# Advanced-Vision-and-Learning-Lab/sparse-view-3dgs-pack

Hardware: AMD Instinct MI355X
Metric: train-step views/s (fwd+bwd) @1M Gaussians 1080p (higher is better)
Workload: dtype f32

## Files before the change

include/gsplat.h:

```cpp
#ifndef GSPLAT_H_INCLUDED
#define GSPLAT_H_INCLUDED

#include <stddef.h>
#include <stdint.h>

#ifdef __cplusplus
extern "C" {
#endif

#define GS_ABI_VERSION 7

#define GS_OK 0
#define GS_E_NULL (-1)
#define GS_E_SHAPE (-2)
#define GS_E_SCRATCH (-3)
#define GS_E_OVERFLOW (-4)
#define GS_E_UNSUPPORTED (-5)

#define GS_TILE_X 16
#define GS_TILE_Y 16
#define GS_NUM_CHANNELS 3

typedef struct GsView {
  int32_t image_height;
// ... 66 lines not shown
int gs_scratch_bytes(int32_t P, int32_t W, int32_t H, int64_t R_capacity, size_t out[3],
                     size_t* backward_workspace_bytes);

int gs_forward_geometry(const GsView* view, const GsGaussians* g, GsScratch* scratch,
                        int32_t* radii, int32_t* num_rendered_host, void* stream);

int gs_forward_render(const GsView* view, const GsGaussians* g, GsScratch* scratch,
                      float* out_color, float* out_invdepth, void* stream);

int gs_forward_bin(const GsView* view, const GsGaussians* g, GsScratch* scratch, uint32_t* status_host, void* stream);

int gs_forward_render_x(const GsView* view, const GsGaussians* g, GsScratch* scratch,
                        float* out_color, float* out_invdepth, float* out_extra, void* stream);

int gs_backward(const GsView* view, const GsGaussians* g, const int32_t* radii,
                const GsScratch* scratch, int64_t num_rendered, const float* dL_dcolor,
                const float* dL_dinvdepth, const GsGrads* grads, void* workspace,
                size_t workspace_bytes, void* stream);

int gs_backward_x(const GsView* view, const GsGaussians* g, const int32_t* radii,
                  const GsScratch* scratch, int64_t num_rendered, const float* dL_dcolor,
                  const float* dL_dinvdepth, const float* dL_dextra_img, const GsGrads* grads,
                  void* workspace, size_t workspace_bytes, void* stream);

int gs_forward_render_fsgs(const GsView* view, const GsGaussians* g, GsScratch* scratch,
                           float* out_color, float* out_depth, float* out_alpha, void* stream);
int gs_backward_fsgs(const GsView* view, const GsGaussians* g, const int32_t* radii,
                     const GsScratch* scratch, int64_t num_rendered, const float* dL_dcolor,
                     const float* dL_ddepth, const float* dL_dalpha, const GsGrads* grads,
                     void* workspace, size_t workspace_bytes, void* stream);

int gs_mark_visible(int32_t P, const float* means3D, const float* viewmatrix,
                    const float* projmatrix, uint8_t* present, void* stream);

int gs_export_geom(const GsScratch* scratch, int32_t P, float* depths, float* means2D ,
                   float* cov3D , float* conic_opacity , float* rgb ,
                   uint8_t* clamped , uint32_t* tiles_touched, uint32_t* point_offsets,
                   void* stream);
int gs_export_binning(const GsScratch* scratch, int64_t num_rendered, uint64_t* keys_sorted,
                      uint32_t* point_list, void* stream);
int gs_export_img(const GsScratch* scratch, int32_t W, int32_t H, float* final_T,
                  uint32_t* n_contrib, uint32_t* ranges , void* stream);

typedef struct GsStepState {
  float* xyz;
  float* features;
  float* opacity;
  float* scaling;
  float* rotation;
  float* m[5];
  float* v[5];
  float lr[6];
  int32_t step[5];
  float beta1, beta2, eps;
  float* max_radii2D;
  float* xyz_gradient_accum;
  float* denom;
  const float* coef_dev;
  const double* rows_override;
  float* grad_out[5];
  float* fail_flag;
  int32_t phase;
  int32_t rows_clean;
  void* phase1_done;
  float* extra;
  float* extra_m;
// ... 237 lines not shown
```

sparse-view-3dgs-pack_amd/csrc/gs_preprocess.hip:

```cpp
#include "gs_common.h"
#include "gs_tilecull.h"
#include "gs_math.h"

template <typename SH>
GS_DEV V3 color_from_sh(int deg, V3 pos, V3 campos, const SH& sh, uint32_t& clamped) {
  V3 dir = pos - campos;
  dir = dir / length3(dir);
  V3 result = SH_C0 * sh(0);
  if (deg > 0) {
    float x = dir.x, y = dir.y, z = dir.z;
    result = result - SH_C1 * y * sh(1) + SH_C1 * z * sh(2) - SH_C1 * x * sh(3);
    if (deg > 1) {
      float xx = x * x, yy = y * y, zz = z * z;
      float xy = x * y, yz = y * z, xz = x * z;
      result = result + SH_C2_0 * xy * sh(4) + SH_C2_1 * yz * sh(5) + SH_C2_2 * (2.0f * zz - xx - yy) * sh(6) +
               SH_C2_3 * xz * sh(7) + SH_C2_4 * (xx - yy) * sh(8);
      if (deg > 2) {
        result = result + SH_C3_0 * y * (3.0f * xx - yy) * sh(9) + SH_C3_1 * xy * z * sh(10) +
                 SH_C3_2 * y * (4.0f * zz - xx - yy) * sh(11) + SH_C3_3 * z * (2.0f * zz - 3.0f * xx - 3.0f * yy) * sh(12) +
                 SH_C3_4 * x * (4.0f * zz - xx - yy) * sh(13) + SH_C3_5 * z * (xx - yy) * sh(14) +
                 SH_C3_6 * x * (xx - 3.0f * yy) * sh(15);
      }
    }
  }
// ... 2 lines not shown
  result.z += 0.5f;
  clamped = (result.x < 0 ? 1u : 0u) | (result.y < 0 ? 2u : 0u) | (result.z < 0 ? 4u : 0u);
  return {fmaxf(result.x, 0.0f), fmaxf(result.y, 0.0f), fmaxf(result.z, 0.0f)};
}

struct ShRegs {
  float f[48];
  __device__ __forceinline__ V3 operator()(int k) const { return {f[3 * k], f[3 * k + 1], f[3 * k + 2]}; }
};
struct ShMem {
  const float* p;
  __device__ __forceinline__ V3 operator()(int k) const { return {p[3 * k], p[3 * k + 1], p[3 * k + 2]}; }
};
struct ShMemSplit {
  const float *dc, *rest;
  __device__ __forceinline__ V3 operator()(int k) const {
    const float* p = k == 0 ? dc : rest + 3 * (k - 1);
    return {p[0], p[1], p[2]};
  }
};

#ifndef GS_LIMIT_TILES_IN_LDS
#define GS_LIMIT_TILES_IN_LDS 0
#endif
#define GS_LIMIT_LDS_MAX_FLOATS (GS_LIMIT_TILES_IN_LDS ? 10240 : 4096)
extern __shared__ float s_limit[];
static inline size_t preprocess_limit_lds_floats(const PreprocessArgs& a) {
  if (!a.tile_depth_limit) return 0;
  const size_t T = (size_t)a.grid_x * a.grid_y, all = depth_limit_floats((uint32_t)a.grid_x, (uint32_t)a.grid_y);
  const size_t want = GS_LIMIT_TILES_IN_LDS ? all : all - T;
  return want <= GS_LIMIT_LDS_MAX_FLOATS ? want : 0;
}

__global__ void __launch_bounds__(GS_BLOCK) preprocess_fwd_kernel(PreprocessArgs a, GeomView g, int lds_floats) {
  const int idx = blockIdx.x * GS_BLOCK + threadIdx.x;
  uint32_t tiles = 0, entries = TB_ENTRIES_UNKNOWN;
  const int T = a.grid_x * a.grid_y;
  int p0 = 0, p1 = 0, p2 = 0, p3 = 0, n_pend = 0;
  uint32_t s0 = 0xFFFFFFFFu, s1 = 0xFFFFFFFFu, s2 = 0xFFFFFFFFu, s3 = 0xFFFFFFFFu, dbits = 0;
  auto bump = [&]() {
    if (n_pend > 0) s0 = atomicAdd(&a.region_count[(size_t)p0 * RG_COUNT_STRIDE], 1u);
    if (n_pend > 1) s1 = atomicAdd(&a.region_count[(size_t)p1 * RG_COUNT_STRIDE], 1u);
    if (n_pend > 2) s2 = atomicAdd(&a.region_count[(size_t)p2 * RG_COUNT_STRIDE], 1u);
    if (n_pend > 3) s3 = atomicAdd(&a.region_count[(size_t)p3 * RG_COUNT_STRIDE], 1u);
    n_pend = 0;
  };
  auto collect = [&]() {
    const uint2 entry = make_uint2(dbits, (uint32_t)idx);
    if (s0 < a.region_cap) a.region_bucket[(size_t)p0 * a.region_cap + s0] = entry;
    if (s1 < a.region_cap) a.region_bucket[(size_t)p1 * a.region_cap + s1] = entry;
    if (s2 < a.region_cap) a.region_bucket[(size_t)p2 * a.region_cap + s2] = entry;
    if (s3 < a.region_cap) a.region_bucket[(size_t)p3 * a.region_cap + s3] = entry;
    s0 = s1 = s2 = s3 = 0xFFFFFFFFu;
  };
  const int lidx = min(idx, a.P - 1);
  typedef const __attribute__((address_space(4))) float* GsConstFloatPtr;
  float vm[16], pm[16], cam[3];
  {
    const GsConstFloatPtr vmp = (GsConstFloatPtr)(uintptr_t)a.viewmatrix, pmp = (GsConstFloatPtr)(uintptr_t)a.projmatrix;
    const GsConstFloatPtr cp = (GsConstFloatPtr)(uintptr_t)a.campos;
#pragma unroll
    for (int k = 0; k < 16; k++) { vm[k] = vmp[k]; pm[k] = pmp[k]; }
    cam[0] = cp[0]; cam[1] = cp[1]; cam[2] = cp[2];
  }
  const bool own_cov = a.cov3D_precomp == nullptr;
  const float* sc_p = own_cov ? a.scales + 3 * (size_t)lidx : a.cov3D_precomp + 6 * (size_t)lidx;
  const float* rq_p = own_cov ? a.rotations + 4 * (size_t)lidx : a.cov3D_precomp + 6 * (size_t)lidx;
  float op_in = a.opacities[lidx];
  V3 p_orig = {a.means3D[3 * (size_t)lidx], a.means3D[3 * (size_t)lidx + 1], a.means3D[3 * (size_t)lidx + 2]};
  V3 sc_in = {sc_p[0], sc_p[1], sc_p[2]};
  V4 rq_in = {rq_p[0], rq_p[1], rq_p[2], rq_p[3]};
  if (lds_floats) {
    const float* src = a.tile_depth_limit + (GS_LIMIT_TILES_IN_LDS ? 0 : T);
    for (int i = threadIdx.x; i < lds_floats; i += GS_BLOCK) s_limit[i] = src[i];
    __syncthreads();
  }
  asm volatile("" : "+v"(op_in), "+v"(sc_in.x), "+v"(sc_in.y), "+v"(sc_in.z), "+v"(rq_in.x), "+v"(rq_in.y), "+v"(rq_in.z),
               "+v"(rq_in.w));
  const GsLdsFloatPtr lds_seg = (GsLdsFloatPtr)s_limit + (GS_LIMIT_TILES_IN_LDS ? T : 0);
  if (idx == 0) g.hdr->pad[HDR_LIMITED] = a.tile_depth_limit ? 1u : 0u;
  if (idx < a.P) {
    Splat sp;
    sp.x = sp.y = sp.depth = sp.invdepth = 0.f;
    sp.cxx = sp.cxy = sp.cyy = sp.opacity = 0.f;
    sp.r = sp.g = sp.b = 0.f;
    sp.extra = 0.f;
    int radius_out = 0;
    sp.rect_min = sp.rect_max = sp.tiles = sp.clamped = 0;
    float cov3D[6] = {0, 0, 0, 0, 0, 0};
    bool write_cov = false;
    do {
      V3 p_view = xform4x3(p_orig, vm);
      if (p_view.z <= 0.2f) break;
      V4 p_hom = xform4x4(p_orig, pm);
      float p_w = 1.0f / (p_hom.w + 0.0000001f);
      V3 p_proj = {p_hom.x * p_w, p_hom.y * p_w, p_hom.z * p_w};

      if (a.cov3D_precomp != nullptr) {
#pragma unroll
        for (int k = 0; k < 6; k++) cov3D[k] = a.cov3D_precomp[(size_t)idx * 6 + k];
      } else {
        const V3 sc = activate_scales(sc_in, a.raw_activations);
        const V4 rq = activate_rotation(rq_in, a.raw_activations);
        M3 S = mat3_cols(1, 0, 0, 0, 1, 0, 0, 0, 1);
        S.c[0][0] = a.scale_modifier * sc.x;
        S.c[1][1] = a.scale_modifier * sc.y;
        S.c[2][2] = a.scale_modifier * sc.z;
        M3 R = quat_to_R(rq);
        M3 Mm = mul3(S, R);
        M3 Sigma = mul3(transpose3(Mm), Mm);
        cov3D[0] = Sigma.c[0][0];
        cov3D[1] = Sigma.c[0][1];
        cov3D[2] = Sigma.c[0][2];
        cov3D[3] = Sigma.c[1][1];
        cov3D[4] = Sigma.c[1][2];
        cov3D[5] = Sigma.c[2][2];
        write_cov = true;
      }
      Cov2DInter ci;
      cov2d_common(p_orig, a.focal_x, a.focal_y, a.tan_fovx, a.tan_fovy, cov3D, vm, ci);
      M3 cv = mul3(mul3(transpose3(ci.T), transpose3(ci.Vrk)), ci.T);
      V3 cov = {cv.c[0][0], cv.c[0][1], cv.c[1][1]};

      const float h_var = 0.3f;
      const float det_cov = cov.x * cov.z - cov.y * cov.y;
      cov.x += h_var;
      cov.z += h_var;
      const float det_cov_plus_h_cov = cov.x * cov.z - cov.y * cov.y;
      float h_convolution_scaling = 1.0f;
      if (a.antialiasing) h_convolution_scaling = sqrtf(fmaxf(0.000025f, det_cov / det_cov_plus_h_cov));
      const float det = det_cov_plus_h_cov;
      if (det == 0.0f) break;
      float det_inv = 1.f / det;
      V3 conic = {cov.z * det_inv, -cov.y * det_inv, cov.x * det_inv};
      float mid = 0.5f * (cov.x + cov.z);
      float lambda1 = mid + sqrtf(fmaxf(0.1f, mid * mid - det));
      float lambda2 = mid - sqrtf(fmaxf(0.1f, mid * mid - det));
      float my_radius = ceilf(3.f * sqrtf(fmaxf(lambda1, lambda2)));
      float pix_x = ndc2pix(p_proj.x, a.W), pix_y = ndc2pix(p_proj.y, a.H);
      uint32_t minx, miny, maxx, maxy;
      const int radius_i = f2i_sat(my_radius);
      get_rect(pix_x, pix_y, radius_i, a.grid_x, a.grid_y, minx, miny, maxx, maxy);
      if ((maxx - minx) * (maxy - miny) == 0) break;

      sp.depth = p_view.z;
      sp.invdepth = 1 / p_view.z;
      radius_out = radius_i;
      sp.extra = a.extra_channel ? load_extra(a.extra_channel, a.extra_gain, idx, a.raw_activations) : 0.f;
      sp.x = pix_x;
      sp.y = pix_y;
      sp.cxx = conic.x; sp.cxy = conic.y; sp.cyy = conic.z;
      sp.opacity = activate_opacity(op_in, a.raw_activations) * h_convolution_scaling;
      sp.rect_min = minx | (miny << 16);
      sp.rect_max = maxx | (maxy << 16);
      if (a.tile_cull == 2) {
        const TileCull tc = tilecull_setup(1, sp.x, sp.y, sp.cxx, sp.cxy, sp.cyy, sp.opacity);
        if (tc.mode != 1) {
          int tx0 = (int)minx, tx1 = (int)maxx, ty0 = (int)miny, ty1 = (int)maxy;
          if (tc.mode == 2) {
            const float big = 1.0e6f;
            const float xl = fminf(fmaxf(sp.x - tc.ex - 1.0f, -big), big), xh = fminf(fmaxf(sp.x + tc.ex + 1.0f, -big), big);
            const float yl = fminf(fmaxf(sp.y - tc.ey - 1.0f, -big), big), yh = fminf(fmaxf(sp.y + tc.ey + 1.0f, -big), big);
            tx0 = max(tx0, (int)floorf(xl * 0.0625f));
            tx1 = min(tx1, (int)floorf(xh * 0.0625f) + 1);
            ty0 = max(ty0, (int)floorf(yl * 0.0625f));
            ty1 = min(ty1, (int)floorf(yh * 0.0625f) + 1);
          }
          if (tx1 > tx0 && ty1 > ty0) {
            const int segs_x = (int)depth_limit_segs_x((uint32_t)a.grid_x);
            dbits = __float_as_uint(sp.depth);
            for (int ry = ty0 >> 2; ry <= (ty1 - 1) >> 2; ry++) {
              for (int rx = tx0 >> 2; rx <= (tx1 - 1) >> 2; rx++) {
                if (a.tile_depth_limit) {
                  float bound = -__builtin_inff();
#pragma unroll
                  for (int k = 0; k < RG_TILES; k++) {
                    const int ty = min(ry * RG_TILES + k, a.grid_y - 1);
                    const float v = lds_floats ? lds_seg[ty * segs_x + rx] : a.tile_depth_limit[(size_t)T + ty * segs_x + rx];
                    bound = fmaxf(bound, v);
                  }
                  if (depth_beyond_limit(sp.depth, bound)) continue;
                }
                const int r = ry * a.rg_x + rx;
                tiles++;
                if (n_pend == 4) { bump(); collect(); }
                p0 = n_pend == 0 ? r : p0;
                p1 = n_pend == 1 ? r : p1;
                p2 = n_pend == 2 ? r : p2;
                p3 = n_pend == 3 ? r : p3;
                n_pend++;
              }
            }
          }
        }
      } else if (a.tile_cull) {
        const TileCull tc = tilecull_setup(1, sp.x, sp.y, sp.cxx, sp.cxy, sp.cyy, sp.opacity);
        if (tc.mode == 0) {
          tiles = (maxy - miny) * (maxx - minx);
          if (!a.tile_depth_limit) entries = tb_rect_entries(minx, miny, maxx, maxy);
        } else if (tc.mode == 2) {
          uint32_t bx0 = 0xFFFFFFFFu, bx1 = 0, by0 = 0xFFFFFFFFu, by1 = 0, tiles_seg = 0;
          uint32_t hull = 0, rowwise = 0, h_lo = 0xFFFFFFFFu, h_hi = 0;
          for (uint32_t ty = miny; ty < maxy; ty++) {
            uint32_t tx0;
            const uint32_t n = tilecull_row_span(tc, ty, minx, maxx, tx0);
            tiles += n;
            if (n) {
              h_lo = min(h_lo, tx0); h_hi = max(h_hi, tx0 + n - 1u);
              rowwise += (tx0 + n - 1u) / RG_TILES - tx0 / RG_TILES + 1u;
            }
            if ((ty % RG_TILES) == RG_TILES - 1u || ty + 1u == maxy) {
              if (h_lo <= h_hi) hull += h_hi / RG_TILES - h_lo / RG_TILES + 1u;
              h_lo = 0xFFFFFFFFu; h_hi = 0;
            }
            if (n && a.tile_depth_limit) {
              bx0 = min(bx0, tx0); bx1 = max(bx1, tx0 + n);
              by0 = min(by0, ty); by1 = ty + 1;
              if (lds_floats) {
                uint32_t t0 = tx0;
                tiles_seg += tilecull_trim_span_segments(lds_seg, (uint32_t)a.grid_x, ty, sp.depth, t0, n);
              }
            }
          }
          if (!a.tile_depth_limit)
            entries = (hull > TB_ENTRIES_MAX || rowwise > TB_ENTRIES_MAX) ? TB_ENTRIES_UNKNOWN : (hull > tiles ? (rowwise | 0x8000u) : hull);
          if (a.tile_depth_limit && tiles) {
            const uint32_t full = tiles;
            uint32_t how = 0;
            if (bx1 - bx0 <= 4u && by1 - by0 <= 4u) {
              uint32_t beyond;
              if (GS_LIMIT_TILES_IN_LDS && lds_floats)
                beyond = depth_limit_box_mask((GsLdsFloatPtr)s_limit, (uint32_t)a.grid_x, bx0, by0, bx1, by1, sp.depth);
              else
                beyond = depth_limit_box_mask(a.tile_depth_limit, (uint32_t)a.grid_x, bx0, by0, bx1, by1, sp.depth);
              if (beyond) {
                tiles = 0;
                for (uint32_t ty = by0; ty < by1; ty++) {
                  uint32_t tx0;
                  const uint32_t n = tilecull_row_span(tc, ty, minx, maxx, tx0);
                  tiles += tilecull_trim_span_mask(beyond, bx0, by0, ty, tx0, n);
                }
                how = 2;
              }
            } else if (lds_floats) {
              tiles = tiles_seg;
              how = 3;
            }
            sp.clamped |= (tiles == 0 ? 1u : (tiles == full ? 0u : how)) << 8;
          }
        }
      } else {
        tiles = (maxy - miny) * (maxx - minx);
        entries = tb_rect_entries(minx, miny, maxx, maxy);
      }
      sp.clamped |= (tiles ? entries : 0u) << 16;
      if (!(a.tile_depth_limit && tiles == 0)) {
        if (a.colors_precomp == nullptr) {
          V3 campos = {cam[0], cam[1], cam[2]};
          V3 rgb;
          uint32_t cl = 0;
          if (a.M == 16 && a.shs_rest) {
            ShRegs sh;
            const float* dc = a.shs + (size_t)idx * 3;
            const float* rest = a.shs_rest + (size_t)idx * 45;
            const int nfl = 3 * (a.D + 1) * (a.D + 1) - 3;
            sh.f[0] = dc[0]; sh.f[1] = dc[1]; sh.f[2] = dc[2];
  #pragma unroll
            for (int k = 0; k < 45; k++) sh.f[3 + k] = k < nfl ? rest[k] : 0.f;
            bump();
            rgb = color_from_sh(a.D, p_orig, campos, sh, cl);
          } else if (a.M == 16) {
            ShRegs sh;
            const float4* src = reinterpret_cast<const float4*>(a.shs + (size_t)idx * 48);
            const int nvec = a.D == 0 ? 1 : (a.D == 1 ? 3 : (a.D == 2 ? 7 : 12));
  #pragma unroll
            for (int k = 0; k < 12; k++) {
              if (k < nvec) {
                float4 v = src[k];
                sh.f[4 * k] = v.x; sh.f[4 * k + 1] = v.y; sh.f[4 * k + 2] = v.z; sh.f[4 * k + 3] = v.w;
              } else {
                sh.f[4 * k] = sh.f[4 * k + 1] = sh.f[4 * k + 2] = sh.f[4 * k + 3] = 0.f;
              }
            }
            bump();
            rgb = color_from_sh(a.D, p_orig, campos, sh, cl);
          } else if (a.shs_rest) {
            bump();
            ShMemSplit sh{a.shs + (size_t)idx * 3, a.shs_rest + (size_t)idx * (a.M - 1) * 3};
            rgb = color_from_sh(a.D, p_orig, campos, sh, cl);
          } else {
            bump();
            ShMem sh{a.shs + (size_t)idx * a.M * 3};
            rgb = color_from_sh(a.D, p_orig, campos, sh, cl);
          }
          sp.r = rgb.x; sp.g = rgb.y; sp.b = rgb.z;
          sp.clamped |= cl;
        } else {
          bump();
          sp.r = a.colors_precomp[3 * idx];
          sp.g = a.colors_precomp[3 * idx + 1];
          sp.b = a.colors_precomp[3 * idx + 2];
        }
      }
      sp.tiles = tiles;
    } while (false);

    const bool write_record = !(a.tile_depth_limit && tiles == 0 && radius_out > 0);
    if (write_record) {
      float4* dst = reinterpret_cast<float4*>(&g.splat[idx]);
      const float4* srcv = reinterpret_cast<const float4*>(&sp);
      dst[0] = srcv[0]; dst[1] = srcv[1]; dst[2] = srcv[2]; dst[3] = srcv[3];
    }
    if (a.cov3D_precomp == nullptr && write_record) {
      float2* cd = reinterpret_cast<float2*>(g.cov3D + (size_t)idx * 6);
      if (!write_cov) { cov3D[0] = cov3D[1] = cov3D[2] = cov3D[3] = cov3D[4] = cov3D[5] = 0.f; }
      cd[0] = make_float2(cov3D[0], cov3D[1]);
      cd[1] = make_float2(cov3D[2], cov3D[3]);
      cd[2] = make_float2(cov3D[4], cov3D[5]);
    }
    g.tiles_touched[idx] = tiles;
    collect();
    if (a.tile_cull != 2) g.depth_keys[idx] = tiles ? __float_as_uint(sp.depth) : 0xFFFFFFFFu;
    a.radii[idx] = radius_out;
  }
  __shared__ uint32_t red[GS_BLOCK / 64];
  uint32_t v = tiles;
#pragma unroll
  for (int off = 32; off >= 1; off >>= 1) v += __shfl_down(v, off, 64);
  if ((threadIdx.x & 63) == 0) red[threadIdx.x >> 6] = v;
  __syncthreads();
  if (threadIdx.x == 0) g.block_sums[blockIdx.x] = red[0] + red[1] + red[2] + red[3];
}

__global__ void __launch_bounds__(1024) scan_block_sums_kernel(GeomView g, int nb, uint32_t P) {
  __shared__ uint32_t wsum[16];
  __shared__ uint32_t carry_s;
  const int tid = threadIdx.x, lane = tid & 63, wid = tid >> 6;
  if (tid == 0) carry_s = 0;
  __syncthreads();
  for (int base = 0; base < nb; base += 1024) {
    int i = base + tid;
    uint32_t v = (i < nb) ? g.block_sums[i] : 0u;
    uint32_t inc = v;
#pragma unroll
    for (int off = 1; off < 64; off <<= 1) {
      uint32_t t = __shfl_up(inc, off, 64);
      if (lane >= off) inc += t;
    }
    if (lane == 63) wsum[wid] = inc;
    __syncthreads();
    uint32_t woff = 0;
    for (int w = 0; w < wid; w++) woff += wsum[w];
    uint32_t carry = carry_s;
    if (i < nb) g.block_sums[i] = carry + woff + inc - v;
    __syncthreads();
    if (tid == 1023) carry_s = carry + woff + inc;
    __syncthreads();
  }
  if (tid == 0) {
    g.block_sums[nb] = carry_s;
    g.hdr->num_rendered = carry_s;
    g.hdr->overflow = 0;
    g.hdr->P = P;
    g.hdr->region_mode = 0;
    g.hdr->pad[HDR_SIDE_CURSOR] = 0;
  }
}

__global__ void __launch_bounds__(GS_BLOCK) mark_visible_kernel(int P, const float* means3D, const float* vm,
                                                                uint8_t* present) {
  const int idx = blockIdx.x * GS_BLOCK + threadIdx.x;
  if (idx >= P) return;
  V3 p = {means3D[3 * idx], means3D[3 * idx + 1], means3D[3 * idx + 2]};
  V3 pv = xform4x3(p, vm);
  present[idx] = !(pv.z <= 0.2f);
}

int launch_preprocess_fwd(const PreprocessArgs& a, const GeomView& g, hipStream_t s) {
  const int nb = (a.P + GS_BLOCK - 1) / GS_BLOCK;
  const size_t lds = preprocess_limit_lds_floats(a);
  hipLaunchKernelGGL(preprocess_fwd_kernel, dim3(nb), dim3(GS_BLOCK), 4 * lds, s, a, g, (int)lds);
  return 0;
}
int launch_scan_block_sums(const GeomView& g, int P, hipStream_t s) {
  const int nb = (P + GS_BLOCK - 1) / GS_BLOCK;
  hipLaunchKernelGGL(scan_block_sums_kernel, dim3(1), dim3(1024), 0, s, g, nb, (uint32_t)P);
  return 0;
}
int launch_mark_visible(int P, const float* means3D, const float* viewmatrix, uint8_t* present, hipStream_t s) {
  hipLaunchKernelGGL(mark_visible_kernel, dim3((P + GS_BLOCK - 1) / GS_BLOCK), dim3(GS_BLOCK), 0, s, P, means3D,
                     viewmatrix, present);
  return 0;
}
```

sparse-view-3dgs-pack_amd/gsplat_amd/capi.py:

```python
import ctypes as C
import os

c_f_p = C.c_void_p


class GsView(C.Structure):
    _fields_ = [
        ("image_height", C.c_int32),
        ("image_width", C.c_int32),
        ("tanfovx", C.c_float),
        ("tanfovy", C.c_float),
        ("scale_modifier", C.c_float),
        ("sh_degree", C.c_int32),
        ("prefiltered", C.c_int32),
        ("antialiasing", C.c_int32),
        ("debug", C.c_int32),
        ("tile_cull", C.c_int32),
        ("bg", C.c_void_p),
        ("viewmatrix", C.c_void_p),
        ("projmatrix", C.c_void_p),
        ("campos", C.c_void_p),
    ]


# ... 77 lines not shown
                ("grad_out_rest", C.c_void_p)]


_P = C.c_void_p
_I32 = C.c_int32
_I64 = C.c_int64
_F = C.c_float
_SZ = C.c_size_t

PROTOTYPES = {
    "abi_version": (C.c_int, []),
    "struct_bytes": (C.c_size_t, [C.c_int32]),
    "build_info": (C.c_char_p, []),
    "scratch_bytes": (C.c_int, [_I32, _I32, _I32, _I64, C.POINTER(_SZ), C.POINTER(_SZ)]),
    "forward_geometry": (C.c_int, [C.POINTER(GsView), C.POINTER(GsGaussians), C.POINTER(GsScratch), _P, _P, _P]),
    "forward_render": (C.c_int, [C.POINTER(GsView), C.POINTER(GsGaussians), C.POINTER(GsScratch), _P, _P, _P]),
    "backward": (C.c_int, [C.POINTER(GsView), C.POINTER(GsGaussians), _P, C.POINTER(GsScratch), _I64, _P, _P,
                           C.POINTER(GsGrads), _P, _SZ, _P]),
    "forward_render_x": (C.c_int, [C.POINTER(GsView), C.POINTER(GsGaussians), C.POINTER(GsScratch), _P, _P, _P, _P]),
    "backward_x": (C.c_int, [C.POINTER(GsView), C.POINTER(GsGaussians), _P, C.POINTER(GsScratch), _I64, _P, _P, _P,
                             C.POINTER(GsGrads), _P, _SZ, _P]),
    "forward_render_fsgs": (C.c_int, [C.POINTER(GsView), C.POINTER(GsGaussians), C.POINTER(GsScratch), _P, _P, _P, _P]),
    "backward_fsgs": (C.c_int, [C.POINTER(GsView), C.POINTER(GsGaussians), _P, C.POINTER(GsScratch), _I64, _P, _P, _P,
                                C.POINTER(GsGrads), _P, _SZ, _P]),
    "step_uninstanced": (C.c_int, [C.POINTER(GsView), C.POINTER(GsGaussians), _P, C.POINTER(GsScratch),
                                   C.POINTER(GsStepState), _P]),
    "backward_step": (C.c_int, [C.POINTER(GsView), C.POINTER(GsGaussians), _P, C.POINTER(GsScratch), _I64, _P, _P,
                                C.POINTER(GsStepState), _P, _SZ, _P]),
    "backward_step_x": (C.c_int, [C.POINTER(GsView), C.POINTER(GsGaussians), _P, C.POINTER(GsScratch), _I64, _P, _P, _P,
                                  C.POINTER(GsStepState), _P, _SZ, _P]),
    "backward_from_rows": (C.c_int, [C.POINTER(GsView), C.POINTER(GsGaussians), _P, C.POINTER(GsScratch), _P, _I32,
                                     C.POINTER(GsGrads), _P, _SZ, _P]),
    "mark_visible": (C.c_int, [_I32, _P, _P, _P, _P, _P]),
    "export_geom": (C.c_int, [C.POINTER(GsScratch), _I32, _P, _P, _P, _P, _P, _P, _P, _P, _P]),
    "export_binning": (C.c_int, [C.POINTER(GsScratch), _I64, _P, _P, _P]),
    "export_img": (C.c_int, [C.POINTER(GsScratch), _I32, _I32, _P, _P, _P, _P]),
    "export_tile_order": (C.c_int, [C.POINTER(GsScratch), _I32, _I32, _P, _P]),
    "export_tile_stop_depth": (C.c_int, [C.POINTER(GsScratch), _I32, _I32, _P, _P]),
    "forward_status": (C.c_int, [C.POINTER(GsScratch), _P, _P]),
    "forward_tile_order": (C.c_int, [C.POINTER(GsView), C.POINTER(GsScratch), _P]),
    "forward_bin": (C.c_int, [C.POINTER(GsView), C.POINTER(GsGaussians), C.POINTER(GsScratch), _P, _P]),
    "export_binning_region": (C.c_int, [C.POINTER(GsScratch), _I32, _I32, _I64, _P, _P, _P]),
    "debug_blend_stats": (C.c_int, [C.POINTER(GsScratch), _I32, _I32, _I32, _P, _P]),
    "tile_depth_limit_floats": (C.c_size_t, [_I32, _I32]),
    "knn_tmp_bytes": (_SZ, [_I32]),
    "knn_mean_dist2": (C.c_int, [_P, _I32, _P, _P, _SZ, _P]),
    "knn_mean_dist2_idx": (C.c_int, [_P, _I32, _P, _P, _P, _SZ, _P]),
    "grid_encode_tmp_bytes": (_SZ, [_I64, _I32, _I32, _I32, _I64]),
    "grid_encode_fwd": (C.c_int, [_P, _I64, _I32, _P, _I64, _I32, _P, _I32, _F, _I32, _I32, _I32, _I32, _P, _P, _P]),
    "grid_encode_bwd": (C.c_int, [_P, _P, _I64, _I32, _I64, _I32, _P, _I32, _F, _I32, _I32, _I32, _I32, _P, _P, _P, _P,
                                  _SZ, _P]),
    "sh_encode_fwd": (C.c_int, [_P, _I64, _I32, _P, _P]),
    "sh_encode_bwd": (C.c_int, [_P, _P, _I64, _I32, _P, _P]),
    "depth_norm_tmp_bytes": (_SZ, [_I32, _I32, _I32, _I32]),
    "depth_norm_fwd": (C.c_int, [_P, _P, _I32, _I32, _I32, _F, _I32, _P, _P, _P, _P]),
    "depth_norm_bwd": (C.c_int, [_P, _P, _I32, _I32, _I32, _F, _I32, _P, _P, _P, _P]),
    "depth_smooth_fwd": (C.c_int, [_P, _P, _I32, _I32, _I32, _P, _P, _P]),
    "depth_smooth_bwd": (C.c_int, [_P, _P, _I32, _I32, _I32, _P, _P, _P, _P]),
    "dng_depth_reg_fwd": (C.c_int, [_P, _P, _I32, _I32, _I32, _I32, _F, _F, _F, _F, _P, _P, _P, _P, _P]),
    "dng_depth_reg_bwd": (C.c_int, [_P, _P, _I32, _I32, _I32, _I32, _F, _F, _F, _F, _P, _P, _P, _P]),
    "pearson_tmp_bytes": (_SZ, [_I64]),
    "pearson_fwd": (C.c_int, [_P, _P, _I64, _I32, _I32, _P, _P, _P, _P]),
    "pearson_bwd": (C.c_int, [_P, _P, _I64, _I32, _I32, _I32, _P, _P, _P, _P, _P]),
    "l1_fwd": (C.c_int, [_P, _P, _I64, _P, _P]),
    "l1_bwd": (C.c_int, [_P, _P, _I64, _F, _P, _I32, _P]),
    "dwt_haar_fwd": (C.c_int, [_P, _I32, _I32, _I32, _P, _P, _P, _P, _P]),
# ... 18 lines not shown
    "l1_dwt2_fwd_clamp": (C.c_int, [_P, _P, _I32, _I32, _I32, _P, _P, _P, _P]),
    "l1_dwt2_patch_fwd_clamp": (C.c_int, [_P, _P, _I32, _I32, _I32, _I32, _P, _P, _P, _P, _P, _P]),
    "l1_dwt2_patch_bwd": (C.c_int, [_P, _P, _I32, _I32, _I32, _I32, _P, _P, _P, _P, _P, _I32, _P]),
    "l1_dwt2_bwd": (C.c_int, [_P, _P, _I32, _I32, _I32, _P, _P, _P, _I32, _P]),
    "ssim_fwd_sum": (C.c_int, [_P, _P, _I32, _I32, _I32, _I32, _F, _F, _P, _P, _P, _P, _P]),
    "ssim_bwd_uniform": (C.c_int, [_P, _P, _I32, _I32, _I32, _I32, _P, _P, _P, _P, _P, _I32, _P, _P]),
    "lgdwt_combine": (C.c_int, [_P, _P, C.POINTER(GsLgdwtParams), _P, _P]),
    "lgdwt_combine_p": (C.c_int, [_P, _P, _I64, _P, C.POINTER(GsLgdwtParams), _P, _P]),
    "ssim_partials_count": (C.c_int64, [_I32, _I32, _I32, _I32]),
    "ssim_fwd_partials": (C.c_int, [_P, _P, _I32, _I32, _I32, _I32, _F, _F, _P, _P, _P, _P, _P]),
    "lgdwt_fused_fwd": (C.c_int, [_P, _P, _I32, _I32, _I32, _F, _F, _I32, _P, _P, _P, _P, _P, _P, _P]),
    "lgdwt_fused_bwd": (C.c_int, [_P, _P, _I32, _I32, _I32, _I32, _I32, _P, _P, _P, _P, _P, _P, _P]),
    "adam_step": (C.c_int, [_P, _P, _P, _P, _I64, C.POINTER(GsAdamSeg), _I32, _F, _F, _F, _I32, _P]),
    "adam_step_gated": (C.c_int, [_P, _P, _P, _P, _I64, C.POINTER(GsAdamSeg), _I32, _F, _F, _F, _I32, _P, _P]),
    "adam_step_masked": (C.c_int, [_P, _P, _P, _P, _I64, C.POINTER(GsAdamSeg), _I32, _F, _F, _F, _I32, _P, _P, _P]),
    "activations_fwd": (C.c_int, [_P, _P, _P, _I32, _P, _P, _P, _P]),
    "activations_bwd": (C.c_int, [_P, _P, _P, _I32, _P, _P, _P, _P, _P, _P, _P]),
    "densify_stats": (C.c_int, [_P, _P, _I32, _P, _P, _P, _P]),
    "profile_enable": (C.c_int, [_I32]),
    "profile_only": (C.c_int, [_I32]),
    "profile_reset": (C.c_int, []),
    "profile_stage_count": (C.c_int, []),
    "rows_pack": (C.c_int, [_P, _I32, _I32, C.POINTER(C.c_int32), _P, _P, _I32, _P, _P]),
    "rows_unpack": (C.c_int, [_P, _I32, _I32, C.POINTER(C.c_int32), _P, _P, _I32, _P, _P]),
    "export_row_mask": (C.c_int, [C.POINTER(GsScratch), _I32, _P, _P]),
    "profile_stage_name": (C.c_char_p, [_I32]),
    "profile_read": (C.c_int, [C.POINTER(C.c_double), C.POINTER(_I64), _I32]),
    "image_stage_partials_count": (C.c_int64, [_I32, _I32]),
    "image_stage_fwd": (C.c_int, [_P, _P, _P, _I32, _I32, _P, _P]),
    "image_stage_bwd": (C.c_int, [_P, _P, _P, _P, _I32, _I32, _P, _P, _P]),
    "exposure_adam": (C.c_int, [_P, _I64, _I32, _P, _P, _P, _P, _I32, _F, C.c_double, C.c_double, _F, _I32, _P, _P]),
}

DEVICE_ONLY = ("export_row_mask", "backward_step", "backward_step_x", "step_uninstanced", "export_tile_order", "export_tile_stop_depth", "forward_status", "forward_bin", "export_binning_region", "debug_blend_stats", "adam_step_gated", "tile_depth_limit_floats", "profile_enable", "profile_only", "profile_reset", "profile_stage_count", "profile_stage_name", "profile_read",
               "forward_render_x", "backward_x", "forward_tile_order",
               "image_stage_partials_count", "image_stage_fwd", "image_stage_bwd", "exposure_adam",
               "lgdwt_fused_fwd", "lgdwt_fused_bwd",
               "grid_encode_tmp_bytes", "grid_encode_fwd", "grid_encode_bwd", "sh_encode_fwd", "sh_encode_bwd",
               "depth_norm_tmp_bytes", "depth_norm_fwd", "depth_norm_bwd", "depth_smooth_fwd", "depth_smooth_bwd",
               "dng_depth_reg_fwd", "dng_depth_reg_bwd",
               "pearson_tmp_bytes", "pearson_fwd", "pearson_bwd")

ERRORS = {-1: "GS_E_NULL", -2: "GS_E_SHAPE", -3: "GS_E_SCRATCH", -4: "GS_E_OVERFLOW", -5: "GS_E_UNSUPPORTED"}


class GsError(RuntimeError):
    def __init__(self, fn, code):
        self.code = code
        what = ERRORS.get(code, "hipError_t %d" % code if code > 0 else "error %d" % code)
        super().__init__("%s failed: %s" % (fn, what))


class CApi:

    def __init__(self, path, prefix="gs_", optional=()):
        if not os.path.exists(path):
            raise ImportError(
                "gsplat native library not found at %s - build it first (python __graft_entry__.py "
                "or `make -C sparse-view-3dgs-pack_amd/csrc`); there is no fallback path." % path)
        self.path = path
        self.prefix = prefix
        self.lib = C.CDLL(path)
        self.missing = []
        for name, (res, args) in PROTOTYPES.items():
            try:
                f = getattr(self.lib, prefix + name)
            except AttributeError:
# ... 24 lines not shown
```

sparse-view-3dgs-pack_amd/gsplat_amd/raster.py:

```python
import ctypes as C
import os

import torch

from .capi import GsGaussians, GsGrads, GsScratch, GsView

NUM_CHANNELS = 3


def _ptr(t):
    if t is None or t.numel() == 0:
        return None
    return t.data_ptr()


def _prep(t, device):
    if t is None or t.numel() == 0:
        return None
    if t.dtype != torch.float32:
        t = t.float()
    if t.device != device:
        t = t.to(device)
    return t.contiguous()

# ... 283 lines not shown

    SLACK = (1.0, 1.25, 1.6, 2.5)
    SLACK_RELAX_AFTER = 24

    def limits_failed(self, c):
        if c is None:
            return
        c["held"] = 0
        if c["slack_level"] < len(self.SLACK) - 1:
            c["slack_level"] += 1
            c["slack"].fill_(self.SLACK[c["slack_level"]])

    def limits_held(self, c):
        if c is None:
            return
        c["held"] += 1
        if c["held"] >= self.SLACK_RELAX_AFTER and c["slack_level"] > 0:
            c["held"] = 0
            c["slack_level"] -= 1
            c["slack"].fill_(self.SLACK[c["slack_level"]])

    @staticmethod
    def _scratch(geom, img=None, binning=None, capacity=0):
        s = GsScratch()
        s.geom, s.geom_bytes = _ptr(geom), geom.numel()
        if img is not None:
            s.img, s.img_bytes = _ptr(img), img.numel()
        if binning is not None:
            s.binning, s.binning_bytes = _ptr(binning), binning.numel()
        s.binning_capacity = int(capacity)
        return s

    force_rowwise_entries = False
    scratch_fill = None
    output_fill = None
    KEYED_LIMITS = os.environ.get("GS_KEYED_LIMITS", "1") != "0"
    STATUS_IN_RENDER = True

    def _side_stream(self, device):
        side = self._side_streams.get(device.index)
        if side is None:
            side = self._side_streams[device.index] = torch.cuda.Stream(device=device)
        return side
    TWO_PHASE = os.environ.get("GS_TWO_PHASE_STEP", "1") != "0"
    TWO_PHASE_MIN_P = 100_000

    def _two_phase(self, step, P):
        return self.TWO_PHASE and P >= self.TWO_PHASE_MIN_P and not step.grad_out[0]

    def _arms_side_launch(self, step, P):
        return self._two_phase(step, P) and not step.rows_override

    def launch_uninstanced_early(self):
        f = self._last
        if f is None or f.step is None or f.done is not None:
            return False
        f.done = self._launch_uninstanced(f.geom.device, f.view, f.g, f.radii, self._scratch(f.geom, f.img), f.step)
        return True

    def _structs(self, device, bg, means3D, sh, colors_precomp, opacities, scales, rotations, cov3D_precomp, viewmatrix,
                 projmatrix, campos, tanfovx, tanfovy, H, W, scale_modifier, degree, antialiasing, debug, extra=None, raw=False,
                 extra_gain=None, sh_rest=None):
        keep = []
        view = self._view(keep, device, bg, viewmatrix, projmatrix, campos, tanfovx, tanfovy, H, W, scale_modifier, degree,
                          False, antialiasing, debug)
        g = self._gauss(keep, device, means3D, sh, colors_precomp, opacities, scales, rotations, cov3D_precomp, extra, raw=raw,
# ... 501 lines not shown
```

Measured before the change: 1188.

## Distribute large-footprint splat region binning cooperatively across the wavefront

In the preprocess kernel, splats whose footprint covers more than four regions no longer walk those regions serially in their own thread. Each wave builds a prefix sum of region counts in LDS, and all 64 lanes then share the depth-limit tests and the region-count atomics and bucket writes. This is meant to remove the load imbalance where one thread with a huge footprint stalls its whole wave. In exchange it adds LDS use, wave barriers, a binary search per work item and an extra counting pass when depth limits are active. It is on by default, with an env or API toggle.

```diff
diff --git a/include/gsplat.h b/include/gsplat.h
--- a/include/gsplat.h
+++ b/include/gsplat.h
@@ -122,6 +122,8 @@
 
 int gs_mark_visible(int32_t P, const float* means3D, const float* viewmatrix,
                     const float* projmatrix, uint8_t* present, void* stream);
+
+int gs_region_coop(int32_t form);
 
 int gs_export_geom(const GsScratch* scratch, int32_t P, float* depths, float* means2D ,
                    float* cov3D , float* conic_opacity , float* rgb ,
diff --git a/sparse-view-3dgs-pack_amd/csrc/gs_preprocess.hip b/sparse-view-3dgs-pack_amd/csrc/gs_preprocess.hip
--- a/sparse-view-3dgs-pack_amd/csrc/gs_preprocess.hip
+++ b/sparse-view-3dgs-pack_amd/csrc/gs_preprocess.hip
@@ -58,6 +58,19 @@
   return want <= GS_LIMIT_LDS_MAX_FLOATS ? want : 0;
 }
 
+#ifndef GS_REGION_COOP_DEFAULT
+#define GS_REGION_COOP_DEFAULT 1
+#endif
+#define GS_COOP_PAIRS 2
+struct CoopWave {
+  uint32_t pref[64];
+  uint32_t dbits[64];
+  uint32_t r0[64];
+  uint32_t nrx[64];
+  uint32_t tiles[64];
+};
+
+template <bool COOP>
 __global__ void __launch_bounds__(GS_BLOCK) preprocess_fwd_kernel(PreprocessArgs a, GeomView g, int lds_floats) {
   const int idx = blockIdx.x * GS_BLOCK + threadIdx.x;
   uint32_t tiles = 0, entries = TB_ENTRIES_UNKNOWN;
@@ -105,16 +118,103 @@
                "+v"(rq_in.w));
   const GsLdsFloatPtr lds_seg = (GsLdsFloatPtr)s_limit + (GS_LIMIT_TILES_IN_LDS ? T : 0);
   if (idx == 0) g.hdr->pad[HDR_LIMITED] = a.tile_depth_limit ? 1u : 0u;
+  const int segs_x = (int)depth_limit_segs_x((uint32_t)a.grid_x);
+  auto region_bound = [&](int rx, int ry) {
+    float bound = -__builtin_inff();
+#pragma unroll
+    for (int k = 0; k < RG_TILES; k++) {
+      const int ty = min(ry * RG_TILES + k, a.grid_y - 1);
+      const float v = lds_floats ? lds_seg[ty * segs_x + rx] : a.tile_depth_limit[(size_t)T + ty * segs_x + rx];
+      bound = fmaxf(bound, v);
+    }
+    return bound;
+  };
+  Splat sp;
+  sp.x = sp.y = sp.depth = sp.invdepth = 0.f;
+  sp.cxx = sp.cxy = sp.cyy = sp.opacity = 0.f;
+  sp.r = sp.g = sp.b = 0.f;
+  sp.extra = 0.f;
+  int radius_out = 0;
+  sp.rect_min = sp.rect_max = sp.tiles = sp.clamped = 0;
+  float cov3D[6] = {0, 0, 0, 0, 0, 0};
+  bool write_cov = false;
+  bool reached = false;
+  uint32_t big_n = 0, big_r0 = 0, big_nrx = 0;
+
+  auto finish = [&]() {
+    sp.clamped |= (tiles ? entries : 0u) << 16;
+    if (!(a.tile_depth_limit && tiles == 0)) {
+      if (a.colors_precomp == nullptr) {
+        V3 campos = {cam[0], cam[1], cam[2]};
+        V3 rgb;
+        uint32_t cl = 0;
+        if (a.M == 16 && a.shs_rest) {
+          ShRegs sh;
+          const float* dc = a.shs + (size_t)idx * 3;
+          const float* rest = a.shs_rest + (size_t)idx * 45;
+          const int nfl = 3 * (a.D + 1) * (a.D + 1) - 3;
+          sh.f[0] = dc[0]; sh.f[1] = dc[1]; sh.f[2] = dc[2];
+#pragma unroll
+          for (int k = 0; k < 45; k++) sh.f[3 + k] = k < nfl ? rest[k] : 0.f;
+          bump();
+          rgb = color_from_sh(a.D, p_orig, campos, sh, cl);
+        } else if (a.M == 16) {
+          ShRegs sh;
+          const float4* src = reinterpret_cast<const float4*>(a.shs + (size_t)idx * 48);
+          const int nvec = a.D == 0 ? 1 : (a.D == 1 ? 3 : (a.D == 2 ? 7 : 12));
+#pragma unroll
+          for (int k = 0; k < 12; k++) {
+            if (k < nvec) {
+              float4 v = src[k];
+              sh.f[4 * k] = v.x; sh.f[4 * k + 1] = v.y; sh.f[4 * k + 2] = v.z; sh.f[4 * k + 3] = v.w;
+            } else {
+              sh.f[4 * k] = sh.f[4 * k + 1] = sh.f[4 * k + 2] = sh.f[4 * k + 3] = 0.f;
+            }
+          }
+          bump();
+          rgb = color_from_sh(a.D, p_orig, campos, sh, cl);
+        } else if (a.shs_rest) {
+          bump();
+          ShMemSplit sh{a.shs + (size_t)idx * 3, a.shs_rest + (size_t)idx * (a.M - 1) * 3};
+          rgb = color_from_sh(a.D, p_orig, campos, sh, cl);
+        } else {
+          bump();
+          ShMem sh{a.shs + (size_t)idx * a.M * 3};
+          rgb = color_from_sh(a.D, p_orig, campos, sh, cl);
+        }
+        sp.r = rgb.x; sp.g = rgb.y; sp.b = rgb.z;
+        sp.clamped |= cl;
+      } else {
+        bump();
+        sp.r = a.colors_precomp[3 * idx];
+        sp.g = a.colors_precomp[3 * idx + 1];
+        sp.b = a.colors_precomp[3 * idx + 2];
+      }
+    }
+    sp.tiles = tiles;
+  };
+
+  bool write_record = true;
+  auto store_record = [&](int half) {
+    float4* dst = reinterpret_cast<float4*>(&g.splat[idx]);
+    const float4* srcv = reinterpret_cast<const float4*>(&sp);
+    dst[2 * half] = srcv[2 * half]; dst[2 * half + 1] = srcv[2 * half + 1];
+  };
+  auto store_geometry = [&]() {
+    write_record = !(a.tile_depth_limit && tiles == 0 && radius_out > 0);
+    if (write_record) store_record(0);
+    if (a.cov3D_precomp == nullptr && write_record) {
+      float2* cd = reinterpret_cast<float2*>(g.cov3D + (size_t)idx * 6);
+      if (!write_cov) { cov3D[0] = cov3D[1] = cov3D[2] = cov3D[3] = cov3D[4] = cov3D[5] = 0.f; }
+      cd[0] = make_float2(cov3D[0], cov3D[1]);
+      cd[1] = make_float2(cov3D[2], cov3D[3]);
+      cd[2] = make_float2(cov3D[4], cov3D[5]);
+    }
+    g.tiles_touched[idx] = tiles;
+    a.radii[idx] = radius_out;
+  };
+
   if (idx < a.P) {
-    Splat sp;
-    sp.x = sp.y = sp.depth = sp.invdepth = 0.f;
-    sp.cxx = sp.cxy = sp.cyy = sp.opacity = 0.f;
-    sp.r = sp.g = sp.b = 0.f;
-    sp.extra = 0.f;
-    int radius_out = 0;
-    sp.rect_min = sp.rect_max = sp.tiles = sp.clamped = 0;
-    float cov3D[6] = {0, 0, 0, 0, 0, 0};
-    bool write_cov = false;
     do {
       V3 p_view = xform4x3(p_orig, vm);
       if (p_view.z <= 0.2f) break;
@@ -179,7 +279,7 @@
       sp.opacity = activate_opacity(op_in, a.raw_activations) * h_convolution_scaling;
       sp.rect_min = minx | (miny << 16);
       sp.rect_max = maxx | (maxy << 16);
-      if (a.tile_cull == 2) {
+      if (COOP || a.tile_cull == 2) {
         const TileCull tc = tilecull_setup(1, sp.x, sp.y, sp.cxx, sp.cxy, sp.cyy, sp.opacity);
         if (tc.mode != 1) {
           int tx0 = (int)minx, tx1 = (int)maxx, ty0 = (int)miny, ty1 = (int)maxy;
@@ -193,28 +293,25 @@
             ty1 = min(ty1, (int)floorf(yh * 0.0625f) + 1);
           }
           if (tx1 > tx0 && ty1 > ty0) {
-            const int segs_x = (int)depth_limit_segs_x((uint32_t)a.grid_x);
             dbits = __float_as_uint(sp.depth);
-            for (int ry = ty0 >> 2; ry <= (ty1 - 1) >> 2; ry++) {
-              for (int rx = tx0 >> 2; rx <= (tx1 - 1) >> 2; rx++) {
-                if (a.tile_depth_limit) {
-                  float bound = -__builtin_inff();
-#pragma unroll
-                  for (int k = 0; k < RG_TILES; k++) {
-                    const int ty = min(ry * RG_TILES + k, a.grid_y - 1);
-                    const float v = lds_floats ? lds_seg[ty * segs_x + rx] : a.tile_depth_limit[(size_t)T + ty * segs_x + rx];
-                    bound = fmaxf(bound, v);
-                  }
-                  if (depth_beyond_limit(sp.depth, bound)) continue;
+            const int rx0 = tx0 >> 2, rx1 = (tx1 - 1) >> 2, ry0 = ty0 >> 2, ry1 = (ty1 - 1) >> 2;
+            if (COOP && (rx1 - rx0 + 1) * (ry1 - ry0 + 1) > 4) {
+              big_nrx = (uint32_t)(rx1 - rx0 + 1);
+              big_n = big_nrx * (uint32_t)(ry1 - ry0 + 1);
+              big_r0 = (uint32_t)rx0 | (uint32_t)ry0 << 16;
+            } else {
+              for (int ry = ry0; ry <= ry1; ry++) {
+                for (int rx = rx0; rx <= rx1; rx++) {
+                  if (a.tile_depth_limit && depth_beyond_limit(sp.depth, region_bound(rx, ry))) continue;
+                  const int r = ry * a.rg_x + rx;
+                  tiles++;
+                  if (!COOP && n_pend == 4) { bump(); collect(); }
+                  p0 = n_pend == 0 ? r : p0;
+                  p1 = n_pend == 1 ? r : p1;
+                  p2 = n_pend == 2 ? r : p2;
+                  p3 = n_pend == 3 ? r : p3;
+                  n_pend++;
                 }
-                const int r = ry * a.rg_x + rx;
-                tiles++;
-                if (n_pend == 4) { bump(); collect(); }
-                p0 = n_pend == 0 ? r : p0;
-                p1 = n_pend == 1 ? r : p1;
-                p2 = n_pend == 2 ? r : p2;
-                p3 = n_pend == 3 ? r : p3;
-                n_pend++;
               }
             }
           }
@@ -279,76 +376,100 @@
         tiles = (maxy - miny) * (maxx - minx);
         entries = tb_rect_entries(minx, miny, maxx, maxy);
       }
-      sp.clamped |= (tiles ? entries : 0u) << 16;
-      if (!(a.tile_depth_limit && tiles == 0)) {
-        if (a.colors_precomp == nullptr) {
-          V3 campos = {cam[0], cam[1], cam[2]};
-          V3 rgb;
-          uint32_t cl = 0;
-          if (a.M == 16 && a.shs_rest) {
-            ShRegs sh;
-            const float* dc = a.shs + (size_t)idx * 3;
-            const float* rest = a.shs_rest + (size_t)idx * 45;
-            const int nfl = 3 * (a.D + 1) * (a.D + 1) - 3;
-            sh.f[0] = dc[0]; sh.f[1] = dc[1]; sh.f[2] = dc[2];
-  #pragma unroll
-            for (int k = 0; k < 45; k++) sh.f[3 + k] = k < nfl ? rest[k] : 0.f;
-            bump();
-            rgb = color_from_sh(a.D, p_orig, campos, sh, cl);
-          } else if (a.M == 16) {
-            ShRegs sh;
-            const float4* src = reinterpret_cast<const float4*>(a.shs + (size_t)idx * 48);
-            const int nvec = a.D == 0 ? 1 : (a.D == 1 ? 3 : (a.D == 2 ? 7 : 12));
-  #pragma unroll
-            for (int k = 0; k < 12; k++) {
-              if (k < nvec) {
-                float4 v = src[k];
-                sh.f[4 * k] = v.x; sh.f[4 * k + 1] = v.y; sh.f[4 * k + 2] = v.z; sh.f[4 * k + 3] = v.w;
-              } else {
-                sh.f[4 * k] = sh.f[4 * k + 1] = sh.f[4 * k + 2] = sh.f[4 * k + 3] = 0.f;
-              }
-            }
-            bump();
-            rgb = color_from_sh(a.D, p_orig, campos, sh, cl);
-          } else if (a.shs_rest) {
-            bump();
-            ShMemSplit sh{a.shs + (size_t)idx * 3, a.shs_rest + (size_t)idx * (a.M - 1) * 3};
-            rgb = color_from_sh(a.D, p_orig, campos, sh, cl);
-          } else {
-            bump();
-            ShMem sh{a.shs + (size_t)idx * a.M * 3};
-            rgb = color_from_sh(a.D, p_orig, campos, sh, cl);
-          }
-          sp.r = rgb.x; sp.g = rgb.y; sp.b = rgb.z;
-          sp.clamped |= cl;
-        } else {
-          bump();
-          sp.r = a.colors_precomp[3 * idx];
-          sp.g = a.colors_precomp[3 * idx + 1];
-          sp.b = a.colors_precomp[3 * idx + 2];
+      if (COOP) {
+        reached = true;
+        break;
+      }
+      finish();
+    } while (false);
+  }
+
+  __shared__ CoopWave s_coop[COOP ? GS_BLOCK / 64 : 1];
+  CoopWave& cw = s_coop[COOP ? threadIdx.x >> 6 : 0];
+  const uint32_t lane = threadIdx.x & 63u;
+  uint32_t coop_total = 0;
+  uint32_t c_p[GS_COOP_PAIRS], c_s[GS_COOP_PAIRS];
+#pragma unroll
+  for (int j = 0; j < GS_COOP_PAIRS; j++) { c_p[j] = 0; c_s[j] = 0xFFFFFFFFu; }
+  auto wave_sync = [&]() {
+    __builtin_amdgcn_fence(__ATOMIC_RELEASE, "wavefront");
+    __builtin_amdgcn_wave_barrier();
+    __builtin_amdgcn_fence(__ATOMIC_ACQUIRE, "wavefront");
+  };
+  auto coop_pair = [&](uint32_t k, uint32_t& owner, uint32_t& r) {
+    uint32_t o = 0;
+#pragma unroll
+    for (uint32_t step = 32; step; step >>= 1) o += cw.pref[o + step - 1u] <= k ? step : 0u;
+    const uint32_t local = k - (o ? cw.pref[o - 1u] : 0u), nrx = cw.nrx[o], r0 = cw.r0[o];
+    const uint32_t row = local / nrx;
+    const int rx = (int)((r0 & 0xFFFFu) + (local - row * nrx)), ry = (int)((r0 >> 16) + row);
+    owner = o;
+    r = (uint32_t)(ry * a.rg_x + rx);
+    return !(a.tile_depth_limit && depth_beyond_limit(__uint_as_float(cw.dbits[o]), region_bound(rx, ry)));
+  };
+  auto coop_bump = [&](uint32_t base) {
+#pragma unroll
+    for (int j = 0; j < GS_COOP_PAIRS; j++) {
+      const uint32_t k = base + 64u * j + lane;
+      uint32_t o, r;
+      if (k < coop_total && coop_pair(k, o, r)) {
+        c_p[j] = r | o << 26;
+        c_s[j] = atomicAdd(&a.region_count[(size_t)r * RG_COUNT_STRIDE], 1u);
+      }
+    }
+  };
+  auto coop_collect = [&]() {
+#pragma unroll
+    for (int j = 0; j < GS_COOP_PAIRS; j++) {
+      if (c_s[j] < a.region_cap) {
+        const uint32_t o = c_p[j] >> 26, r = c_p[j] & 0x3FFFFFFu;
+        a.region_bucket[(size_t)r * a.region_cap + c_s[j]] = make_uint2(cw.dbits[o], (uint32_t)idx - lane + o);
+      }
+      c_s[j] = 0xFFFFFFFFu;
+    }
+  };
+  if constexpr (COOP) {
+    uint32_t pref = big_n;
+#pragma unroll
+    for (int off = 1; off < 64; off <<= 1) {
+      const uint32_t t = __shfl_up(pref, off, 64);
+      if ((int)lane >= off) pref += t;
+    }
+    coop_total = (uint32_t)__builtin_amdgcn_readlane((int)pref, 63);
+    if (coop_total) {
+      cw.pref[lane] = pref; cw.dbits[lane] = dbits; cw.r0[lane] = big_r0; cw.nrx[lane] = big_nrx; cw.tiles[lane] = 0;
+      wave_sync();
+      if (a.tile_depth_limit) {
+        for (uint32_t base = 0; base < coop_total; base += 64u) {
+          const uint32_t k = base + lane;
+          uint32_t o, r;
+          if (k < coop_total && coop_pair(k, o, r)) atomicAdd(&cw.tiles[o], 1u);
         }
-      }
-      sp.tiles = tiles;
-    } while (false);
-
-    const bool write_record = !(a.tile_depth_limit && tiles == 0 && radius_out > 0);
-    if (write_record) {
-      float4* dst = reinterpret_cast<float4*>(&g.splat[idx]);
-      const float4* srcv = reinterpret_cast<const float4*>(&sp);
-      dst[0] = srcv[0]; dst[1] = srcv[1]; dst[2] = srcv[2]; dst[3] = srcv[3];
-    }
-    if (a.cov3D_precomp == nullptr && write_record) {
-      float2* cd = reinterpret_cast<float2*>(g.cov3D + (size_t)idx * 6);
-      if (!write_cov) { cov3D[0] = cov3D[1] = cov3D[2] = cov3D[3] = cov3D[4] = cov3D[5] = 0.f; }
-      cd[0] = make_float2(cov3D[0], cov3D[1]);
-      cd[1] = make_float2(cov3D[2], cov3D[3]);
-      cd[2] = make_float2(cov3D[4], cov3D[5]);
-    }
-    g.tiles_touched[idx] = tiles;
+        wave_sync();
+        if (big_n) tiles = cw.tiles[lane];
+      } else {
+        tiles = big_n ? big_n : tiles;
+      }
+      uint32_t base = 0;
+      for (; base + 64u * GS_COOP_PAIRS < coop_total; base += 64u * GS_COOP_PAIRS) {
+        coop_bump(base);
+        coop_collect();
+      }
+      coop_bump(base);
+    }
+    if (idx < a.P) store_geometry();
+    if (reached) finish();
+    if (idx < a.P) {
+      if (write_record) store_record(1);
+      collect();
+    }
+  } else if (idx < a.P) {
+    store_geometry();
+    if (write_record) store_record(1);
     collect();
     if (a.tile_cull != 2) g.depth_keys[idx] = tiles ? __float_as_uint(sp.depth) : 0xFFFFFFFFu;
-    a.radii[idx] = radius_out;
-  }
+  }
+  if constexpr (COOP) coop_collect();
   __shared__ uint32_t red[GS_BLOCK / 64];
   uint32_t v = tiles;
 #pragma unroll
@@ -402,10 +523,28 @@
   present[idx] = !(pv.z <= 0.2f);
 }
 
+static int g_region_coop = -1;
+static int region_coop_form() {
+  if (g_region_coop < 0) {
+    const char* e = getenv("GS_REGION_COOP");
+    g_region_coop = e ? (atoi(e) != 0 ? 1 : 0) : GS_REGION_COOP_DEFAULT;
+  }
+  return g_region_coop;
+}
+extern "C" int gs_region_coop(int32_t form) {
+  if (form >= 0) g_region_coop = form ? 1 : 0;
+  return region_coop_form();
+}
+
 int launch_preprocess_fwd(const PreprocessArgs& a, const GeomView& g, hipStream_t s) {
   const int nb = (a.P + GS_BLOCK - 1) / GS_BLOCK;
   const size_t lds = preprocess_limit_lds_floats(a);
-  hipLaunchKernelGGL(preprocess_fwd_kernel, dim3(nb), dim3(GS_BLOCK), 4 * lds, s, a, g, (int)lds);
+  const bool coop = a.tile_cull == 2 && region_coop_form() && a.rg_x <= 0xFFFF && a.rg_y <= 0xFFFF &&
+                    (long long)a.rg_x * a.rg_y <= (1ll << 26);
+  if (coop)
+    hipLaunchKernelGGL(preprocess_fwd_kernel<true>, dim3(nb), dim3(GS_BLOCK), 4 * lds, s, a, g, (int)lds);
+  else
+    hipLaunchKernelGGL(preprocess_fwd_kernel<false>, dim3(nb), dim3(GS_BLOCK), 4 * lds, s, a, g, (int)lds);
   return 0;
 }
 int launch_scan_block_sums(const GeomView& g, int P, hipStream_t s) {
diff --git a/sparse-view-3dgs-pack_amd/gsplat_amd/capi.py b/sparse-view-3dgs-pack_amd/gsplat_amd/capi.py
--- a/sparse-view-3dgs-pack_amd/gsplat_amd/capi.py
+++ b/sparse-view-3dgs-pack_amd/gsplat_amd/capi.py
@@ -133,6 +133,7 @@
     "backward_from_rows": (C.c_int, [C.POINTER(GsView), C.POINTER(GsGaussians), _P, C.POINTER(GsScratch), _P, _I32,
                                      C.POINTER(GsGrads), _P, _SZ, _P]),
     "mark_visible": (C.c_int, [_I32, _P, _P, _P, _P, _P]),
+    "region_coop": (C.c_int, [_I32]),
     "export_geom": (C.c_int, [C.POINTER(GsScratch), _I32, _P, _P, _P, _P, _P, _P, _P, _P, _P]),
     "export_binning": (C.c_int, [C.POINTER(GsScratch), _I64, _P, _P, _P]),
     "export_img": (C.c_int, [C.POINTER(GsScratch), _I32, _I32, _P, _P, _P, _P]),
@@ -217,7 +218,7 @@
     "exposure_adam": (C.c_int, [_P, _I64, _I32, _P, _P, _P, _P, _I32, _F, C.c_double, C.c_double, _F, _I32, _P, _P]),
 }
 
-DEVICE_ONLY = ("export_row_mask", "backward_step", "backward_step_x", "step_uninstanced", "export_tile_order", "export_tile_stop_depth", "forward_status", "forward_bin", "export_binning_region", "debug_blend_stats", "adam_step_gated", "tile_depth_limit_floats", "profile_enable", "profile_only", "profile_reset", "profile_stage_count", "profile_stage_name", "profile_read",
+DEVICE_ONLY = ("export_row_mask", "backward_step", "backward_step_x", "step_uninstanced", "export_tile_order", "export_tile_stop_depth", "forward_status", "forward_bin", "export_binning_region", "region_coop", "debug_blend_stats", "adam_step_gated", "tile_depth_limit_floats", "profile_enable", "profile_only", "profile_reset", "profile_stage_count", "profile_stage_name", "profile_read",
                "forward_render_x", "backward_x", "forward_tile_order",
                "image_stage_partials_count", "image_stage_fwd", "image_stage_bwd", "exposure_adam",
                "lgdwt_fused_fwd", "lgdwt_fused_bwd",
diff --git a/sparse-view-3dgs-pack_amd/gsplat_amd/raster.py b/sparse-view-3dgs-pack_amd/gsplat_amd/raster.py
--- a/sparse-view-3dgs-pack_amd/gsplat_amd/raster.py
+++ b/sparse-view-3dgs-pack_amd/gsplat_amd/raster.py
@@ -339,6 +339,15 @@
         return s
 
     force_rowwise_entries = False
+
+    @property
+    def region_coop(self):
+        return bool(self.api.raw("region_coop")(-1))
+
+    @region_coop.setter
+    def region_coop(self, on):
+        self.api.raw("region_coop")(int(bool(on)))
+
     scratch_fill = None
     output_fill = None
     KEYED_LIMITS = os.environ.get("GS_KEYED_LIMITS", "1") != "0"
```

Result: faster. 1232 (median of 6 runs) (+3.6%).
